# ateme-developers/SVT-AV1-1

Hardware: AMD Instinct MI355X
Metric: 64x64 SAD-search blocks/sec (higher is better)
Workload: dtype u8; 1 GPU; configs[1]: 64x64 full-pel SAD hierarchical ME (centre check + HME L0/L1/L2 + 64x64-area full-pel search of 85 square PUs), 1080p 8-bit, one reference list

## Files before the change

### svt-av1-1_amd/csrc/me_fullpel_common.h

```cpp
#pragma once
#include <hip/hip_runtime.h>
#include <stdint.h>

#include "me_kernels.h"
#include "me_sad_common.h"

namespace svthip {

constexpr int kPitch = SVTHIP_FULLPEL_LDS_PITCH;

struct FullpelDesc {
    int src_off, ref_off, xo, yo, sw, sh, n_xg;
    uint32_t inv_xg;
};

__device__ __forceinline__ FullpelDesc fullpel_decode_desc(const int32_t* d)
{
    FullpelDesc D;
    D.src_off = __builtin_amdgcn_readfirstlane(d[0]);
    D.ref_off = __builtin_amdgcn_readfirstlane(d[1]);
    D.xo = __builtin_amdgcn_readfirstlane(d[2]);
    D.yo = __builtin_amdgcn_readfirstlane(d[3]);
    D.sw = __builtin_amdgcn_readfirstlane(d[4]);
    D.sh = __builtin_amdgcn_readfirstlane(d[5]);
    D.n_xg = (D.sw + 15) >> 4;
    D.inv_xg = (65536u + (uint32_t)D.n_xg - 1u) / (uint32_t)D.n_xg;
    return D;
}

template <int PITCH, int IMAGE1 = 0>
__device__ __forceinline__ void stage_window(uint8_t* win, const uint8_t* base, uint32_t ref_stride, int sw, int sh, int tid)
{
    const int rows = sh + 63;
    const int ndw_valid = (sw + 63 + 3) >> 2;
    constexpr int q_row = PITCH >> 4;
    const int total = rows * q_row;
    auto slot = [](const uint8_t* p, int left) {
        uint32_t t[4] = {0u, 0u, 0u, 0u};
        if (left >= 4) {
            const unaligned_u32x4 u = *reinterpret_cast<const unaligned_u32x4*>(p);
            t[0] = u.v[0]; t[1] = u.v[1]; t[2] = u.v[2]; t[3] = u.v[3];
        } else if (left > 0) {
#pragma unroll
            for (int k = 0; k < 3; k++)
                if (k < left) t[k] = reinterpret_cast<const unaligned_u32*>(p + 4 * k)->v;
        }
        return make_uint4(t[0], t[1], t[2], t[3]);
    };
    for (int i = tid; i < total; i += 256) {
        const int r = i / q_row;
        const int c4 = i - r * q_row;
        const uint8_t* p = base + (size_t)r * ref_stride + 16 * c4;
        const int left = ndw_valid - 4 * c4;
        reinterpret_cast<uint4*>(win)[i] = slot(p, left);
        if constexpr (IMAGE1 != 0) reinterpret_cast<uint4*>(win + IMAGE1)[i] = slot(p + 4, left - 1);
    }
}

__device__ __forceinline__ bool fullpel_raster_item(int it, int lane, int n_items, int n_xg, uint32_t inv_xg, int& y, int& xg)
{
    int pg = it * 64 + lane;
    const bool lane_valid = pg < n_items;
    if (!lane_valid) pg = 0;
    y = (int)(((uint32_t)pg * inv_xg) >> 16);
    xg = pg - y * n_xg;
    return lane_valid;
}
__device__ __forceinline__ uint32_t fullpel_idx0(int y, int xg) { return (uint32_t)(y * 128 + 16 * xg); }

__device__ __forceinline__ uint32_t track_class8(uint32_t best, const uint64_t (&acc)[4], const uint32_t* idx, uint32_t himask)
{
    const uint32_t mlo = pk_min_u16(pk_min_u16((uint32_t)acc[0], (uint32_t)acc[1]), pk_min_u16((uint32_t)acc[2], (uint32_t)acc[3]));
    const uint32_t mhi = pk_min_u16(pk_min_u16((uint32_t)(acc[0] >> 32), (uint32_t)(acc[1] >> 32)),
                                    pk_min_u16((uint32_t)(acc[2] >> 32), (uint32_t)(acc[3] >> 32)));
    return track4(best, pack64(mlo, mhi), idx, himask);
}

__device__ __forceinline__ void widen_sums32(const uint32_t (&s16lo)[4][4], const uint32_t (&s16hi)[4][4], uint32_t (&s32acc)[16])
{
#pragma unroll
    for (int q = 0; q < 4; q++) {
        const uint32_t a_lo = s16lo[0][q] + s16lo[1][q], b_lo = s16lo[2][q] + s16lo[3][q];
        const uint32_t a_hi = s16hi[0][q] + s16hi[1][q], b_hi = s16hi[2][q] + s16hi[3][q];
        s32acc[4 * q + 0] = (a_lo & 0xffffu) + (b_lo & 0xffffu);
        s32acc[4 * q + 1] = (a_lo >> 16) + (b_lo >> 16);
        s32acc[4 * q + 2] = (a_hi & 0xffffu) + (b_hi & 0xffffu);
        s32acc[4 * q + 3] = (a_hi >> 16) + (b_hi >> 16);
    }
}

__device__ __forceinline__ uint32_t track32(uint32_t best, const uint32_t (&s32acc)[16], const uint32_t (&idx)[16])
{
#pragma unroll
    for (int i = 0; i < 16; i += 2) {
        uint32_t k0 = (s32acc[i] << 14) | idx[i];
        uint32_t k1 = (s32acc[i + 1] << 14) | idx[i + 1];
        best = min3u(best, k0, k1);
    }
    return best;
}

__device__ __forceinline__ void pu8_origin(int p, int& px, int& py)
{
    const int zz = p >> 2, k = p & 3;
    px = 16 * (zz & 1) + 8 * (k & 1);
    py = 16 * (zz >> 1) + 8 * (k >> 1);
}

template <int PITCH>
__device__ __forceinline__ void resolve_class8(const uint8_t* win, uint32_t key, const uint32_t (&rs)[4][2], int lane, int Q, int xo, int yo,
                                               uint32_t* osad, uint32_t* omv)
{
    const int p = lane >> 2, q = lane & 3;
    const uint32_t s = key >> 16, id = key & 0xffffu;
    const int y = (int)(id >> 7), xb = (int)(id & 0x70u);
    int px, py;
    pu8_origin(p, px, py);
    const uint8_t* wp = win + (y + 32 * (Q >> 1) + py) * PITCH + xb + 4 * q + 32 * (Q & 1) + px;
    uint64_t a = 0;
#pragma unroll
    for (int r = 0; r < 4; r++) {
        const uint32_t* w = reinterpret_cast<const uint32_t*>(wp + 2 * r * PITCH);
        const uint32_t w0 = w[0], w1 = w[1], w2 = w[2];
        a = __builtin_amdgcn_qsad_pk_u16_u8(pack64(w0, w1), rs[r][0], a);
        a = __builtin_amdgcn_qsad_pk_u16_u8(pack64(w1, w2), rs[r][1], a);
    }
    const uint32_t lo = (uint32_t)a, hi = (uint32_t)(a >> 32);
    uint32_t first = (lo & 0xffffu) == s ? 0u : (lo >> 16) == s ? 1u : (hi & 0xffffu) == s ? 2u : (hi >> 16) == s ? 3u : 64u;
    first += 4u * (uint32_t)q;
    first = min(first, (uint32_t)__shfl_xor((int)first, 1));
    first = min(first, (uint32_t)__shfl_xor((int)first, 2));
    if (q == 0) {
        const int pu = 21 + 16 * Q + p;
        osad[pu] = 2u * s;
        omv[pu] = mv_word(xo + xb + (int)first, yo + y);
    }
}

__device__ __forceinline__ void store_pu(uint32_t* osad, uint32_t* omv, int pu, uint32_t raw, uint32_t id, int xo, int yo)
{
    osad[pu] = 2u * raw;
    omv[pu] = mv_word(xo + (int)(id & 127u), yo + (int)(id >> 7));
}

__device__ __forceinline__ void merge_best64(unsigned long long* best64_lds, uint32_t raw, uint32_t idx, int lane)
{
    const unsigned long long k64 = wave_min_u64(((unsigned long long)raw << 32) | idx);
    if (lane == 0) atomicMin(best64_lds, k64);
}
__device__ __forceinline__ void read_best64(const unsigned long long* best64_lds, uint32_t& raw, uint32_t& id)
{
    const unsigned long long k = *best64_lds;
    raw = (uint32_t)(k >> 32);
    id = (uint32_t)k;
}

}
```

### svt-av1-1_amd/csrc/me_fullpel_impl.h

```cpp
#pragma once
#include <hip/hip_runtime.h>
#include <stdint.h>

#include "me_fullpel_common.h"
#include "me_fullpel_img2.h"
#include "me_kernels.h"
#include "me_wave_reduce.h"

namespace svthip {
namespace {

constexpr int kPitch2 = SVTHIP_FULLPEL_IMG2_PITCH;
constexpr int kImage1 = SVTHIP_FULLPEL_IMG2_ROWS * SVTHIP_FULLPEL_IMG2_PITCH;
constexpr unsigned long long kRowLut = 0xFEAB6732DC894510ull;

template <bool CLS, bool IMG2 = false>
__device__ __forceinline__ void fullpel85_sb(const uint8_t* __restrict__ src_plane, uint32_t src_stride,
                                             const uint8_t* __restrict__ ref_plane, uint32_t ref_stride, const int32_t* d, uint32_t sbi,
                                             uint32_t* __restrict__ out_sad, uint32_t* __restrict__ out_mv, uint8_t* smem)
{
    uint32_t* xch = reinterpret_cast<uint32_t*>(smem);
    unsigned long long* best64_lds = reinterpret_cast<unsigned long long*>(smem + 16384);
    uint8_t* win = smem + 16384 + 64;
    static_assert(!IMG2 || CLS, "the two-image form is a form of the class loop");
    constexpr int P = IMG2 ? kPitch2 : kPitch;

    const int tid = threadIdx.x;
    const int lane = tid & 63;
    const int Q = __builtin_amdgcn_readfirstlane(tid >> 6);
    const int Qx = Q & 1, Qy = Q >> 1;

    const FullpelDesc D = fullpel_decode_desc(d);
    const int xo = D.xo, yo = D.yo, sw = D.sw, sh = D.sh, n_xg = D.n_xg;

    stage_window<P, IMG2 ? kImage1 : 0>(win, ref_plane + D.ref_off, ref_stride, sw, sh, tid);
    if (tid == 0) *best64_lds = ~0ull;
    __syncthreads();

    const uint32_t* src4 = reinterpret_cast<const uint32_t*>(src_plane + D.src_off + (size_t)(32 * Qy) * src_stride + 32 * Qx);
    const int sstride4 = src_stride >> 2;

    uint32_t rsv[4][2] = {{0, 0}, {0, 0}, {0, 0}, {0, 0}};
    if constexpr (CLS) {
        const int p = lane >> 2, zz = p >> 2, k = p & 3, px = 16 * (zz & 1) + 8 * (k & 1), py = 16 * (zz >> 1) + 8 * (k >> 1);
        const uint32_t* sp = src4 + (size_t)py * sstride4 + (px >> 2);
#pragma unroll
        for (int r = 0; r < 4; r++) {
            rsv[r][0] = sp[(size_t)(2 * r) * sstride4];
            rsv[r][1] = sp[(size_t)(2 * r) * sstride4 + 1];
        }
    }

    uint32_t best8[16], best16[4], best32 = 0xffffffffu;
#pragma unroll
    for (int i = 0; i < 16; i++) best8[i] = 0xffffffffu;
#pragma unroll
    for (int i = 0; i < 4; i++) best16[i] = 0xffffffffu;
    uint32_t best64_raw = 0xffffffffu, best64_idx = 0;

    const uint32_t himask = 0xffff0000u;
    const int n_items = n_xg * sh;
    const int n_iter = IMG2 ? (sh + 15) >> 4 : (n_items + 63) >> 6;
    const int lane_row = (int)((kRowLut >> (4 * (lane >> 2))) & 15u);

    for (int it = 0; it < n_iter; it++) {
        int y, xg;
        bool lane_valid;
        if constexpr (IMG2) {
            y = 16 * it + lane_row;
            xg = lane & 3;
            lane_valid = y < sh;
            if (!lane_valid) y = 0;
        } else {
            lane_valid = fullpel_raster_item(it, lane, n_items, n_xg, D.inv_xg, y, xg);
        }

        uint32_t idx[16];
        const uint32_t idx0 = fullpel_idx0(y, xg);
        if (IMG2 || (sw & 15) == 0) {
#pragma unroll
            for (int i = 0; i < 16; i++) idx[i] = idx0 + (uint32_t)i;
        } else {
#pragma unroll
            for (int i = 0; i < 16; i++) idx[i] = (16 * xg + i < sw) ? idx0 + (uint32_t)i : 0xffffffffu;
        }

        uint32_t s16lo[4][4], s16hi[4][4];

        const uint8_t* wbase = win + (y + 32 * Qy) * P + 16 * xg + 32 * Qx;

        uint4 An, Bn, Cn = make_uint4(0, 0, 0, 0), Dn = make_uint4(0, 0, 0, 0);
        uint32_t Sn[4];
        {
            if constexpr (IMG2) {
                An = lds_read_b128(wbase);
                Bn = lds_read_b128(wbase + 16);
                Cn = lds_read_b128(wbase + kImage1);
                Dn = lds_read_b128(wbase + kImage1 + 16);
            } else {
                An = *reinterpret_cast<const uint4*>(wbase);
                Bn = *reinterpret_cast<const uint4*>(wbase + 16);
            }
#pragma unroll
            for (int h = 0; h < 4; h++) Sn[h] = src4[h];
        }
#pragma unroll
        for (int zz = 0; zz < 4; zz++) {
            uint64_t acc[4][4];

#pragma unroll
            for (int r8 = 0; r8 < 8; r8++) {
                const uint4 A = An, B = Bn, Cw = Cn, Dw = Dn;
                const uint32_t W[8] = {A.x, A.y, A.z, A.w, B.x, B.y, B.z, B.w};
                const uint32_t S[4] = {Sn[0], Sn[1], Sn[2], Sn[3]};
                const uint64_t WP[7] = {pack64(W[0], W[1]), IMG2 ? pack64(Cw.x, Cw.y) : pack64(W[1], W[2]), pack64(W[2], W[3]),
                                        IMG2 ? pack64(Cw.z, Cw.w) : pack64(W[3], W[4]), pack64(W[4], W[5]),
                                        IMG2 ? pack64(Dw.x, Dw.y) : pack64(W[5], W[6]), pack64(W[6], W[7])};
                asm volatile("" ::"v"(A.x), "v"(A.y), "v"(A.z), "v"(A.w), "v"(B.x), "v"(B.y), "v"(B.z), "v"(B.w), "s"(S[0]), "s"(S[1]), "s"(S[2]), "s"(S[3]));
                if constexpr (IMG2) asm volatile("" ::"v"(Cw.x), "v"(Cw.y), "v"(Cw.z), "v"(Cw.w), "v"(Dw.x), "v"(Dw.y), "v"(Dw.z), "v"(Dw.w));
                __builtin_amdgcn_sched_barrier(0);
                {
                    const int nstep = zz * 8 + r8 + 1;
                    if (nstep < 32) {
                        const int nzz = nstep >> 3, nr8 = nstep & 7, nC = nzz & 1, nR = nzz >> 1;
                        const uint8_t* p = wbase + (16 * nR + 2 * nr8) * P + 16 * nC;
                        if constexpr (IMG2) {
                            An = lds_read_b128(p);
                            Bn = lds_read_b128(p + 16);
                            Cn = lds_read_b128(p + kImage1);
                            Dn = lds_read_b128(p + kImage1 + 16);
                        } else {
                            An = *reinterpret_cast<const uint4*>(p);
                            Bn = *reinterpret_cast<const uint4*>(p + 16);
                        }
                        const uint32_t* srow = src4 + (16 * nR + 2 * nr8) * sstride4 + 4 * nC;
#pragma unroll
                        for (int h = 0; h < 4; h++) Sn[h] = srow[h];
                    }
                    __builtin_amdgcn_sched_barrier(0);
                }
                const int krow = (r8 >> 2) * 2;
#pragma unroll
                for (int q = 0; q < 4; q++)
#pragma unroll
                    for (int h = 0; h < 4; h++) {
                        const int k = krow + (h >> 1);
                        const bool first = ((r8 & 3) == 0) && ((h & 1) == 0);
                        acc[k][q] = __builtin_amdgcn_qsad_pk_u16_u8(WP[q + h], S[h], first ? 0ull : acc[k][q]);
                    }
            }

#pragma unroll
            for (int k = 0; k < 4; k++) {
                if constexpr (CLS) {
                    best8[4 * zz + k] = track_class8(best8[4 * zz + k], acc[k], &idx[0], himask);
                } else {
#pragma unroll
                    for (int q = 0; q < 4; q++) best8[4 * zz + k] = track4(best8[4 * zz + k], acc[k][q], &idx[4 * q], himask);
                }
            }

#pragma unroll
            for (int q = 0; q < 4; q++) {
                const uint32_t lo = (uint32_t)acc[0][q] + (uint32_t)acc[1][q] + (uint32_t)acc[2][q] + (uint32_t)acc[3][q];
                const uint32_t hi = (uint32_t)(acc[0][q] >> 32) + (uint32_t)(acc[1][q] >> 32) +
                                    (uint32_t)(acc[2][q] >> 32) + (uint32_t)(acc[3][q] >> 32);
                best16[zz] = track4(best16[zz], pack64(lo, hi), &idx[4 * q], himask);
                s16lo[zz][q] = lo;
                s16hi[zz][q] = hi;
            }
        }

        uint32_t s32acc[16];
        widen_sums32(s16lo, s16hi, s32acc);
        best32 = track32(best32, s32acc, idx);

        __syncthreads();
        {
            uint4* dst = reinterpret_cast<uint4*>(xch + Q * 1024 + lane * 4);
#pragma unroll
            for (int q = 0; q < 4; q++) dst[q * 64] = make_uint4(s32acc[4 * q], s32acc[4 * q + 1], s32acc[4 * q + 2], s32acc[4 * q + 3]);
        }
        __syncthreads();
        {
            uint4 s = make_uint4(0, 0, 0, 0);
#pragma unroll
            for (int w = 0; w < 4; w++) {
                const uint4 v = *reinterpret_cast<const uint4*>(xch + w * 1024 + Q * 256 + lane * 4);
                s.x += v.x; s.y += v.y; s.z += v.z; s.w += v.w;
            }
            const uint32_t sv[4] = {s.x, s.y, s.z, s.w};
            const int xbase = 16 * xg + 4 * Q;
            const uint32_t ibase = (uint32_t)(y * 128 + xbase);
#pragma unroll
            for (int j = 0; j < 4; j++) {
                const bool better = (sv[j] < best64_raw) && lane_valid && (xbase + j < sw);
                best64_raw = better ? sv[j] : best64_raw;
                best64_idx = better ? (ibase + j) : best64_idx;
            }
        }
    }

    uint32_t* osad = out_sad + (size_t)85 * sbi;
    uint32_t* omv = out_mv + (size_t)85 * sbi;

    const uint32_t g8 = wave_min_scatter<16>(best8, lane);
    const uint32_t top[8] = {best16[0], best16[1], best16[2], best16[3], best32, 0xffffffffu, 0xffffffffu, 0xffffffffu};
    const uint32_t g16 = wave_min_scatter<8, 5>(top, lane);

    if constexpr (CLS) {
        resolve_class8<P>(win, (uint32_t)__shfl((int)g8, lane >> 2), rsv, lane, Q, xo, yo, osad, omv);
    }
    if (lane < 21 && !(CLS && lane < 16)) {
        const uint32_t key = lane < 16 ? g8 : g16;
        const int pu = lane < 16 ? 21 + 16 * Q + lane : lane < 20 ? 5 + 4 * Q + (lane - 16) : 1 + Q;
        const uint32_t raw = lane == 20 ? key >> 14 : key >> 16, id = key & 0x3fffu;
        store_pu(osad, omv, pu, raw, id, xo, yo);
    }
    merge_best64(best64_lds, best64_raw, best64_idx, lane);
    __syncthreads();
    if (tid == 0) {
        uint32_t raw, id;
        read_best64(best64_lds, raw, id);
        store_pu(osad, omv, 0, raw, id, xo, yo);
    }
}

}
}
```

### svt-av1-1_amd/csrc/me_sad_common.h

```cpp
#pragma once
#include <hip/hip_runtime.h>
#include <stdint.h>

namespace svthip {

__device__ __forceinline__ uint64_t pack64(uint32_t lo, uint32_t hi) { return ((uint64_t)hi << 32) | lo; }

typedef uint32_t u32x4_t __attribute__((ext_vector_type(4)));
__device__ __forceinline__ uint4 lds_read_b128(const uint8_t* p)
{
    const u32x4_t v = *(const volatile __attribute__((address_space(3))) u32x4_t*)p;
    return make_uint4(v.x, v.y, v.z, v.w);
}

struct __attribute__((packed, aligned(1))) unaligned_u32 { uint32_t v; };
struct __attribute__((packed, aligned(1))) unaligned_u32x4 { uint32_t v[4]; };

__device__ __forceinline__ uint32_t min3u(uint32_t a, uint32_t b, uint32_t c)
{
    uint32_t r;
    asm("v_min3_u32 %0, %1, %2, %3" : "=v"(r) : "v"(a), "v"(b), "v"(c));
    return r;
}

__device__ __forceinline__ uint32_t track4(uint32_t best, uint64_t acc, const uint32_t* idx, uint32_t himask)
{
    const uint32_t lo = (uint32_t)acc, hi = (uint32_t)(acc >> 32);
    uint32_t k0 = (lo << 16) | idx[0];
    uint32_t k1 = (lo & himask) | idx[1];
    uint32_t k2 = (hi << 16) | idx[2];
    uint32_t k3 = (hi & himask) | idx[3];
    best = min3u(best, k0, k1);
    best = min3u(best, k2, k3);
    return best;
}

__device__ __forceinline__ uint32_t pk_min_u16(uint32_t a, uint32_t b)
{
    uint32_t r;
    asm("v_pk_min_u16 %0, %1, %2" : "=v"(r) : "v"(a), "v"(b));
    return r;
}

__device__ __forceinline__ uint32_t wave_min_u32(uint32_t v)
{
#pragma unroll
    for (int m = 1; m < 64; m <<= 1) {
        uint32_t o = __shfl_xor(v, m);
        v = o < v ? o : v;
    }
    return v;
}

__device__ __forceinline__ unsigned long long wave_min_u64(unsigned long long v)
{
#pragma unroll
    for (int m = 1; m < 64; m <<= 1) {
        unsigned long long o = __shfl_xor(v, m);
        v = o < v ? o : v;
    }
    return v;
}

__device__ __forceinline__ uint32_t mv_word(int x, int y)
{
    return ((uint32_t)(uint16_t)(y * 4) << 16) | (uint32_t)(uint16_t)(x * 4);
}

}
```

Measured before the change: 9.778 million blocks/s.

## Track per-item minima in hot loop and resolve 8/16/32 MV offsets afterwards

In the classed path the inner loop no longer tracks a per-candidate index for every SAD. It reduces each item's 16 candidates to one packed-u16 minimum and keys it with the item base index, for the 8x8, 16x16 and 32x32 PUs alike. The exact x offset is found after the loop by recomputing SADs at the winning item and matching the value, with cross-lane shuffle sums for 16x16 and 32x32. The 64x64 best is also packed into a single 32-bit key with a u32 wave min when the window fits, replacing the 64-bit raw/idx tracking. This trims ALU work in the hot loop at the cost of a longer epilogue and ties resolved to the first match.

```diff
diff --git a/svt-av1-1_amd/csrc/me_fullpel_common.h b/svt-av1-1_amd/csrc/me_fullpel_common.h
--- a/svt-av1-1_amd/csrc/me_fullpel_common.h
+++ b/svt-av1-1_amd/csrc/me_fullpel_common.h
@@ -100,6 +100,29 @@
     return best;
 }
 
+
+__device__ __forceinline__ uint32_t track_item16(uint32_t best, const uint32_t (&d)[8], uint32_t idx0, uint32_t himask)
+{
+    const uint32_t m = pk_min_u16_tree(pk_min_u16_tree(pk_min_u16_tree(d[0], d[1]), pk_min_u16_tree(d[2], d[3])),
+                                       pk_min_u16_tree(pk_min_u16_tree(d[4], d[5]), pk_min_u16_tree(d[6], d[7])));
+    return min3u(best, (m << 16) | idx0, (m & himask) | idx0);
+}
+
+__device__ __forceinline__ uint32_t track_item32(uint32_t best, const uint32_t (&s32acc)[16], uint32_t idx0)
+{
+    uint32_t m = min3u(s32acc[0], s32acc[1], s32acc[2]);
+#pragma unroll
+    for (int i = 3; i < 15; i += 2) m = min3u(m, s32acc[i], s32acc[i + 1]);
+    return min3u(best, (m << 14) | idx0, (s32acc[15] << 14) | idx0);
+}
+
+__device__ __forceinline__ uint32_t track_quad64(uint32_t best, const uint32_t (&sv)[4], int y, int x0)
+{
+    const uint32_t i0 = (uint32_t)(y * 64 + x0);
+    best = min3u(best, (sv[0] << 12) | i0, (sv[1] << 12) | (i0 + 1u));
+    return min3u(best, (sv[2] << 12) | (i0 + 2u), (sv[3] << 12) | (i0 + 3u));
+}
+
 __device__ __forceinline__ void pu8_origin(int p, int& px, int& py)
 {
     const int zz = p >> 2, k = p & 3;
@@ -137,6 +160,55 @@
     }
 }
 
+template <int PITCH>
+__device__ __forceinline__ void resolve_items(const uint8_t* win, uint32_t key8, uint32_t key16, uint32_t key32, const uint32_t (&rs)[4][2],
+                                              int lane, int Q, int xo, int yo, uint32_t* osad, uint32_t* omv)
+{
+    const int p = lane >> 2, q = lane & 3;
+    int px, py;
+    pu8_origin(p, px, py);
+    const uint8_t* wpart = win + (32 * (Q >> 1) + py) * PITCH + 4 * q + 32 * (Q & 1) + px;
+#pragma unroll
+    for (int pass = 0; pass < 3; pass++) {
+        const uint32_t key = pass == 0 ? key8 : pass == 1 ? key16 : key32;
+        const int kbits = pass == 2 ? 14 : 16;
+        const uint32_t s = key >> kbits, id = key & ((1u << kbits) - 1u);
+        const int y = (int)(id >> 7), xb = (int)(id & 0x70u);
+        const uint8_t* wp = wpart + y * PITCH + xb;
+        uint64_t a = 0;
+#pragma unroll
+        for (int r = 0; r < 4; r++) {
+            const uint32_t* w = reinterpret_cast<const uint32_t*>(wp + 2 * r * PITCH);
+            const uint32_t w0 = w[0], w1 = w[1], w2 = w[2];
+            a = __builtin_amdgcn_qsad_pk_u16_u8(pack64(w0, w1), rs[r][0], a);
+            a = __builtin_amdgcn_qsad_pk_u16_u8(pack64(w1, w2), rs[r][1], a);
+        }
+        uint32_t lo = (uint32_t)a, hi = (uint32_t)(a >> 32);
+        if (pass >= 1) {
+            lo += (uint32_t)__shfl_xor((int)lo, 4); hi += (uint32_t)__shfl_xor((int)hi, 4);
+            lo += (uint32_t)__shfl_xor((int)lo, 8); hi += (uint32_t)__shfl_xor((int)hi, 8);
+        }
+        if (pass == 2) {
+            lo += (uint32_t)__shfl_xor((int)lo, 16); hi += (uint32_t)__shfl_xor((int)hi, 16);
+        }
+        uint32_t c[4] = {lo & 0xffffu, lo >> 16, hi & 0xffffu, hi >> 16};
+        if (pass == 2) {
+#pragma unroll
+            for (int j = 0; j < 4; j++) c[j] += (uint32_t)__shfl_xor((int)c[j], 32);
+        }
+        uint32_t first = c[0] == s ? 0u : c[1] == s ? 1u : c[2] == s ? 2u : c[3] == s ? 3u : 64u;
+        first += 4u * (uint32_t)q;
+        first = min(first, (uint32_t)__shfl_xor((int)first, 1));
+        first = min(first, (uint32_t)__shfl_xor((int)first, 2));
+        const int pu_lanes = pass == 0 ? 4 : pass == 1 ? 16 : 64;
+        if ((lane & (pu_lanes - 1)) == 0) {
+            const int pu = pass == 0 ? 21 + 16 * Q + p : pass == 1 ? 5 + 4 * Q + (p >> 2) : 1 + Q;
+            osad[pu] = 2u * s;
+            omv[pu] = mv_word(xo + xb + (int)first, yo + y);
+        }
+    }
+}
+
 __device__ __forceinline__ void store_pu(uint32_t* osad, uint32_t* omv, int pu, uint32_t raw, uint32_t id, int xo, int yo)
 {
     osad[pu] = 2u * raw;
@@ -154,5 +226,16 @@
     raw = (uint32_t)(k >> 32);
     id = (uint32_t)k;
 }
-
-}
+__device__ __forceinline__ void merge_best64_key(unsigned long long* best64_lds, uint32_t key, int lane)
+{
+    const uint32_t k = wave_min_u32(key);
+    if (lane == 0) atomicMin(reinterpret_cast<uint32_t*>(best64_lds), k);
+}
+__device__ __forceinline__ void read_best64_key(const unsigned long long* best64_lds, uint32_t& raw, uint32_t& id)
+{
+    const uint32_t k = *reinterpret_cast<const uint32_t*>(best64_lds);
+    raw = k >> 12;
+    id = ((k & 0xfc0u) << 1) | (k & 63u);
+}
+
+}
diff --git a/svt-av1-1_amd/csrc/me_fullpel_impl.h b/svt-av1-1_amd/csrc/me_fullpel_impl.h
--- a/svt-av1-1_amd/csrc/me_fullpel_impl.h
+++ b/svt-av1-1_amd/csrc/me_fullpel_impl.h
@@ -57,6 +57,7 @@
 #pragma unroll
     for (int i = 0; i < 4; i++) best16[i] = 0xffffffffu;
     uint32_t best64_raw = 0xffffffffu, best64_idx = 0;
+    const bool key64 = CLS && (IMG2 || (sw <= 64 && sh <= 64));
 
     const uint32_t himask = 0xffff0000u;
     const int n_items = n_xg * sh;
@@ -77,12 +78,14 @@
 
         uint32_t idx[16];
         const uint32_t idx0 = fullpel_idx0(y, xg);
-        if (IMG2 || (sw & 15) == 0) {
-#pragma unroll
-            for (int i = 0; i < 16; i++) idx[i] = idx0 + (uint32_t)i;
-        } else {
-#pragma unroll
-            for (int i = 0; i < 16; i++) idx[i] = (16 * xg + i < sw) ? idx0 + (uint32_t)i : 0xffffffffu;
+        if constexpr (!CLS) {
+            if ((sw & 15) == 0) {
+#pragma unroll
+                for (int i = 0; i < 16; i++) idx[i] = idx0 + (uint32_t)i;
+            } else {
+#pragma unroll
+                for (int i = 0; i < 16; i++) idx[i] = (16 * xg + i < sw) ? idx0 + (uint32_t)i : 0xffffffffu;
+            }
         }
 
         uint32_t s16lo[4][4], s16hi[4][4];
@@ -153,7 +156,9 @@
 #pragma unroll
             for (int k = 0; k < 4; k++) {
                 if constexpr (CLS) {
-                    best8[4 * zz + k] = track_class8(best8[4 * zz + k], acc[k], &idx[0], himask);
+                    const uint32_t d[8] = {(uint32_t)acc[k][0], (uint32_t)(acc[k][0] >> 32), (uint32_t)acc[k][1], (uint32_t)(acc[k][1] >> 32),
+                                           (uint32_t)acc[k][2], (uint32_t)(acc[k][2] >> 32), (uint32_t)acc[k][3], (uint32_t)(acc[k][3] >> 32)};
+                    best8[4 * zz + k] = track_item16(best8[4 * zz + k], d, idx0, himask);
                 } else {
 #pragma unroll
                     for (int q = 0; q < 4; q++) best8[4 * zz + k] = track4(best8[4 * zz + k], acc[k][q], &idx[4 * q], himask);
@@ -165,15 +170,20 @@
                 const uint32_t lo = (uint32_t)acc[0][q] + (uint32_t)acc[1][q] + (uint32_t)acc[2][q] + (uint32_t)acc[3][q];
                 const uint32_t hi = (uint32_t)(acc[0][q] >> 32) + (uint32_t)(acc[1][q] >> 32) +
                                     (uint32_t)(acc[2][q] >> 32) + (uint32_t)(acc[3][q] >> 32);
-                best16[zz] = track4(best16[zz], pack64(lo, hi), &idx[4 * q], himask);
+                if constexpr (!CLS) best16[zz] = track4(best16[zz], pack64(lo, hi), &idx[4 * q], himask);
                 s16lo[zz][q] = lo;
                 s16hi[zz][q] = hi;
             }
+            if constexpr (CLS) {
+                const uint32_t d[8] = {s16lo[zz][0], s16hi[zz][0], s16lo[zz][1], s16hi[zz][1], s16lo[zz][2], s16hi[zz][2], s16lo[zz][3], s16hi[zz][3]};
+                best16[zz] = track_item16(best16[zz], d, idx0, himask);
+            }
         }
 
         uint32_t s32acc[16];
         widen_sums32(s16lo, s16hi, s32acc);
-        best32 = track32(best32, s32acc, idx);
+        if constexpr (CLS) best32 = track_item32(best32, s32acc, idx0);
+        else best32 = track32(best32, s32acc, idx);
 
         __syncthreads();
         {
@@ -191,12 +201,16 @@
             }
             const uint32_t sv[4] = {s.x, s.y, s.z, s.w};
             const int xbase = 16 * xg + 4 * Q;
-            const uint32_t ibase = (uint32_t)(y * 128 + xbase);
-#pragma unroll
-            for (int j = 0; j < 4; j++) {
-                const bool better = (sv[j] < best64_raw) && lane_valid && (xbase + j < sw);
-                best64_raw = better ? sv[j] : best64_raw;
-                best64_idx = better ? (ibase + j) : best64_idx;
+            if (key64) {
+                best64_raw = track_quad64(best64_raw, sv, y, xbase);
+            } else {
+                const uint32_t ibase = (uint32_t)(y * 128 + xbase);
+#pragma unroll
+                for (int j = 0; j < 4; j++) {
+                    const bool better = (sv[j] < best64_raw) && lane_valid && (xbase + j < sw);
+                    best64_raw = better ? sv[j] : best64_raw;
+                    best64_idx = better ? (ibase + j) : best64_idx;
+                }
             }
         }
     }
@@ -209,19 +223,21 @@
     const uint32_t g16 = wave_min_scatter<8, 5>(top, lane);
 
     if constexpr (CLS) {
-        resolve_class8<P>(win, (uint32_t)__shfl((int)g8, lane >> 2), rsv, lane, Q, xo, yo, osad, omv);
-    }
-    if (lane < 21 && !(CLS && lane < 16)) {
+        resolve_items<P>(win, (uint32_t)__shfl((int)g8, lane >> 2), (uint32_t)__shfl((int)g16, lane >> 4), (uint32_t)__shfl((int)g16, 4), rsv,
+                         lane, Q, xo, yo, osad, omv);
+    } else if (lane < 21) {
         const uint32_t key = lane < 16 ? g8 : g16;
         const int pu = lane < 16 ? 21 + 16 * Q + lane : lane < 20 ? 5 + 4 * Q + (lane - 16) : 1 + Q;
         const uint32_t raw = lane == 20 ? key >> 14 : key >> 16, id = key & 0x3fffu;
         store_pu(osad, omv, pu, raw, id, xo, yo);
     }
-    merge_best64(best64_lds, best64_raw, best64_idx, lane);
+    if (key64) merge_best64_key(best64_lds, best64_raw, lane);
+    else merge_best64(best64_lds, best64_raw, best64_idx, lane);
     __syncthreads();
     if (tid == 0) {
         uint32_t raw, id;
-        read_best64(best64_lds, raw, id);
+        if (key64) read_best64_key(best64_lds, raw, id);
+        else read_best64(best64_lds, raw, id);
         store_pu(osad, omv, 0, raw, id, xo, yo);
     }
 }
diff --git a/svt-av1-1_amd/csrc/me_sad_common.h b/svt-av1-1_amd/csrc/me_sad_common.h
--- a/svt-av1-1_amd/csrc/me_sad_common.h
+++ b/svt-av1-1_amd/csrc/me_sad_common.h
@@ -42,6 +42,12 @@
     return r;
 }
 
+typedef unsigned short u16x2_t __attribute__((ext_vector_type(2)));
+__device__ __forceinline__ uint32_t pk_min_u16_tree(uint32_t a, uint32_t b)
+{
+    return __builtin_bit_cast(uint32_t, __builtin_elementwise_min(__builtin_bit_cast(u16x2_t, a), __builtin_bit_cast(u16x2_t, b)));
+}
+
 __device__ __forceinline__ uint32_t wave_min_u32(uint32_t v)
 {
 #pragma unroll
```

Result: faster. 9.957 million blocks/s (median of 6 runs) (+1.8%).
